# SamsungLabs/nb-asr

Measured on AMD Instinct MI355X. Metric: utterances_per_sec, higher is better.
Workload: dtype f32

## Files before the change

nb_asr_amd/csrc/gemm_pointwise.hip:

```cpp
#include "storage.h"

namespace nbasr {

typedef float floatx4 __attribute__((ext_vector_type(4)));
typedef _Float16 pw_h2 __attribute__((ext_vector_type(2)));

constexpr int PW_M = 128, PW_N = 256, PW_K = 32;
constexpr int PW_THREADS = 512;

__device__ __forceinline__ float pw_load(const float* p) { return *p; }
__device__ __forceinline__ float pw_load(const bf16_t* p) { return __uint_as_float(static_cast<unsigned>(p->bits) << 16); }
__device__ __forceinline__ void pw_store(float* p, float v) { *p = v; }
__device__ __forceinline__ void pw_store(bf16_t* p, float v) { p->bits = static_cast<unsigned short>(pack_bf16x2(v, 0.f) & 0xffffu); }

template <int TERMS>
struct PwSteps {
    static constexpr int NS = TERMS;
    static constexpr int A_STEP = TERMS * 2 * 2 * PW_M * 16;
    static constexpr int X_STEP = TERMS * 2 * 2 * PW_N * 16;
    static constexpr int LDS = 2 * (A_STEP + X_STEP);
};

struct PwF16x2 : PwSteps<2> {
    typedef _Float16 vec8 __attribute__((ext_vector_type(8)));
    typedef float act_t;
    static constexpr bool SCALED = true;
    static constexpr bool ORDER_BY_HOST = true;
    static constexpr int LD_ALIGN = 4, PROJECTION_LD_ALIGN = 1;
    __device__ static __forceinline__ void split2(float a, float b, unsigned (&d)[NS]) {
        const _Float16 ha = static_cast<_Float16>(a), hb = static_cast<_Float16>(b);
        d[0] = __builtin_bit_cast(unsigned, pw_h2{ha, hb});
        d[1] = __builtin_bit_cast(unsigned, pw_h2{static_cast<_Float16>((a - static_cast<float>(ha)) * 2048.f),
                                                  static_cast<_Float16>((b - static_cast<float>(hb)) * 2048.f)});
    }
    __device__ static __forceinline__ floatx4 mfma(vec8 a, vec8 b, floatx4 c) { return __builtin_amdgcn_mfma_f32_16x16x32_f16(a, b, c, 0, 0, 0); }
};

struct PwBf16 : PwSteps<1> {
    typedef __bf16 vec8 __attribute__((ext_vector_type(8)));
    typedef bf16_t act_t;
    static constexpr bool SCALED = false;
    static constexpr bool ORDER_BY_HOST = false;
    static constexpr int LD_ALIGN = 8, PROJECTION_LD_ALIGN = 8;
    __device__ static __forceinline__ void split2(float a, float b, unsigned (&d)[NS]) { d[0] = pack_bf16x2(a, b); }
    __device__ static __forceinline__ floatx4 mfma(vec8 a, vec8 b, floatx4 c) { return __builtin_amdgcn_mfma_f32_16x16x32_bf16(a, b, c, 0, 0, 0); }
};

__host__ __device__ inline void pw_pow2(float absmax, int target, float& scale, float& inv)
{
    unsigned bits;
    __builtin_memcpy(&bits, &absmax, 4);
    const int e = static_cast<int>((bits >> 23) & 0xffu);
    int k = (bits & 0x7fffffffu) ? (127 + target) - e : 0;
    k = k > 126 ? 126 : (k < -126 ? -126 : k);
    const unsigned sb = static_cast<unsigned>(127 + k) << 23, ib = static_cast<unsigned>(127 - k) << 23;
    __builtin_memcpy(&scale, &sb, 4);
    __builtin_memcpy(&inv, &ib, 4);
}

__global__ __launch_bounds__(256) void pw_row_scales_kernel(const float* __restrict__ w, float* __restrict__ scales, int c_out,
                                                            int c_in, int rows)
{
    __shared__ float s_max[4];
    const int co = blockIdx.x;
    float m = 0.f;
    if (co < c_out)
        for (int i = threadIdx.x; i < c_in; i += 256) m = fmaxf(m, fabsf(w[static_cast<size_t>(co) * c_in + i]));
#pragma unroll
    for (int d = 32; d >= 1; d >>= 1) m = fmaxf(m, __shfl_xor(m, d));
    if ((threadIdx.x & 63) == 0) s_max[threadIdx.x >> 6] = m;
    __syncthreads();
    if (threadIdx.x == 0) {
        float scale, inv;
        pw_pow2(fmaxf(fmaxf(s_max[0], s_max[1]), fmaxf(s_max[2], s_max[3])), 13, scale, inv);
        scales[co] = scale;
        scales[rows + co] = inv;
    }
}

template <class P>
__global__ __launch_bounds__(256) void pw_pack_weights_kernel(const float* __restrict__ w, unsigned short* __restrict__ wp,
                                                              const float* __restrict__ row_scale, int c_out, int c_in,
                                                              int n_mt, int n_ks)
{
    const long long total = static_cast<long long>(n_mt) * n_ks * PW_M * PW_K;
    for (long long i = static_cast<long long>(blockIdx.x) * blockDim.x + threadIdx.x; i < total;
         i += static_cast<long long>(gridDim.x) * blockDim.x) {
        long long e = i;
        const int ci_l = e % PW_K; e /= PW_K;
        const int co_l = e % PW_M; e /= PW_M;
        const int ks = e % n_ks; e /= n_ks;
        const int mt = static_cast<int>(e);
        const int co = mt * PW_M + co_l, ci = ks * PW_K + ci_l;
        float v = 0.f;
        if (co < c_out && ci < c_in) v = P::SCALED ? w[static_cast<size_t>(co) * c_in + ci] * row_scale[co] : w[static_cast<size_t>(co) * c_in + ci];
        unsigned d[P::NS];
        P::split2(v, 0.f, d);
        const int blk = ci_l >> 4, half = (ci_l >> 3) & 1, c8 = ci_l & 7;
        const size_t step = static_cast<size_t>(mt) * n_ks + ks;
        const size_t base = step * (P::A_STEP / 2) + ((static_cast<size_t>(blk) * 2 + half) * PW_M + co_l) * 8 + c8;
#pragma unroll
        for (int s = 0; s < P::NS; ++s) wp[base + s * (P::A_STEP / 2 / P::NS)] = static_cast<unsigned short>(d[s] & 0xffffu);
    }
}


template <bool LNX, class T>
__device__ __forceinline__ void pw_fetch32(const T* __restrict__ x, int c_in, int frames, int ld, const LnRef& ln, float (&v)[PW_K])
{
    const int ci0 = blockIdx.y * PW_K, b = blockIdx.z;
    const int t = blockIdx.x * PW_N + threadIdx.x;
    const bool live = t < frames;
    const T* __restrict__ xb = x + static_cast<size_t>(b) * c_in * ld + t;
    float mean = 0.f, rstd = 0.f;
    if (LNX && live) {
        const float* st = ln.stats + static_cast<size_t>(b) * 2 * ld;
        mean = st[t]; rstd = st[ld + t];
    }
#pragma unroll
    for (int c = 0; c < PW_K; ++c) {
        const int ci = ci0 + c;
        v[c] = (live && ci < c_in) ? pw_load(xb + static_cast<size_t>(ci) * ld) : 0.f;
    }
    if (LNX) {
#pragma unroll
        for (int c = 0; c < PW_K; ++c) {
            const int ci = ci0 + c;
            if (live && ci < c_in) v[c] = ln_apply(v[c], mean, rstd, ln.gamma[ci], ln.beta[ci]);
        }
    }
}

template <bool LNX>
__global__ __launch_bounds__(256) void pw_tile_max_kernel(const float* __restrict__ x, float* __restrict__ partial, int c_in,
                                                          int frames, int ld, int n_ks, const LnRef ln)
{
    __shared__ float s_max[4];
    float v[PW_K];
    pw_fetch32<LNX>(x, c_in, frames, ld, ln, v);
    float m = 0.f;
#pragma unroll
    for (int c = 0; c < PW_K; ++c) m = fmaxf(m, fabsf(v[c]));
#pragma unroll
    for (int d = 32; d >= 1; d >>= 1) m = fmaxf(m, __shfl_xor(m, d));
    if ((threadIdx.x & 63) == 0) s_max[threadIdx.x >> 6] = m;
    __syncthreads();
    if (threadIdx.x == 0)
        partial[(static_cast<size_t>(blockIdx.z) * gridDim.x + blockIdx.x) * n_ks + blockIdx.y] = fmaxf(fmaxf(s_max[0], s_max[1]), fmaxf(s_max[2], s_max[3]));
}

template <class P, bool LNX>
__global__ __launch_bounds__(256) void pw_presplit_kernel(const typename P::act_t* __restrict__ x, unsigned char* __restrict__ image,
                                                          float* __restrict__ inv_scale, const float* __restrict__ partial,
                                                          int c_in, int frames, int ld, int n_ks, const LnRef ln)
{
    const int nt = blockIdx.x, ks = blockIdx.y, b = blockIdx.z;
    const int lane_t = threadIdx.x;
    float v[PW_K];
    pw_fetch32<LNX>(x, c_in, frames, ld, ln, v);
    float scale = 1.f;
    if constexpr (P::SCALED) {
        const float* __restrict__ pt = partial + (static_cast<size_t>(b) * gridDim.x + nt) * n_ks;
        float tile_max = 0.f;
        for (int i = threadIdx.x & 63; i < n_ks; i += 64) tile_max = fmaxf(tile_max, pt[i]);
#pragma unroll
        for (int d = 32; d >= 1; d >>= 1) tile_max = fmaxf(tile_max, __shfl_xor(tile_max, d));
        float inv;
        pw_pow2(tile_max, 14, scale, inv);
        if (threadIdx.x == 0 && ks == 0) inv_scale[static_cast<size_t>(b) * gridDim.x + nt] = inv;
    }
    unsigned char* step = image + ((static_cast<size_t>(b) * gridDim.x + nt) * n_ks + ks) * P::X_STEP;
#pragma unroll
    for (int bh = 0; bh < 4; ++bh) {
        u4v term[P::NS];
#pragma unroll
        for (int q = 0; q < 4; ++q) {
            const float v0 = v[bh * 8 + 2 * q], v1 = v[bh * 8 + 2 * q + 1];
            unsigned d[P::NS];
            if constexpr (P::SCALED) P::split2(v0 * scale, v1 * scale, d);
            else P::split2(v0, v1, d);
#pragma unroll
            for (int s = 0; s < P::NS; ++s) term[s][q] = d[s];
        }
        unsigned char* row = step + (bh * PW_N + lane_t) * 16;
#pragma unroll
        for (int s = 0; s < P::NS; ++s) *reinterpret_cast<u4v*>(row + s * (P::X_STEP / P::NS)) = term[s];
    }
}

template <class P>
struct PointwiseArgs {
    const unsigned char* image; const float* x_inv; const unsigned char* wp; const float* w_inv;
    const float* bias; const float* bias2;
    const typename P::act_t* s0; const typename P::act_t* s1; const typename P::act_t* s2;
    void* y;
    int c_out, frames, ld_out, n_ks, n_mt, n_nt, batch;
    int n_major;
    int row_stride_t, row_stride_b;
    LnRef ln_s0;
};

template <class P, bool SWAP, bool RELU>
__global__ __launch_bounds__(PW_THREADS, 2) void pw_gemm_kernel(const PointwiseArgs<P> a)
{
    typedef typename P::vec8 vec8;
    typedef typename P::act_t act_t;
    constexpr int NS = P::NS, A_STEP = P::A_STEP, X_STEP = P::X_STEP;
    extern __shared__ __attribute__((aligned(16))) unsigned char smem[];
    unsigned char* const Abuf = smem;
    unsigned char* const Xbuf = smem + 2 * A_STEP;

    const int nwg = gridDim.x, id = blockIdx.x;
    const int xq = nwg >> 3, xr = nwg & 7, xcd = id & 7;
    const int L = (xcd < xr ? xcd * (xq + 1) : xr * (xq + 1) + (xcd - xr) * xq) + (id >> 3);
    int mt_i, b, nt_i;
    if (!P::ORDER_BY_HOST || a.n_major) {
        const int ntg = L / a.n_mt;
        mt_i = L - ntg * a.n_mt;
        b = ntg / a.n_nt;
        nt_i = ntg - b * a.n_nt;
    } else {
        const int per_m = a.n_nt * a.batch;
        mt_i = L / per_m;
        const int rem = L - mt_i * per_m;
        b = rem / a.n_nt;
        nt_i = rem - b * a.n_nt;
    }
    const int m0 = mt_i * PW_M, n0 = nt_i * PW_N;

    const int tid = threadIdx.x, lane = tid & 63;
    const int wave = __builtin_amdgcn_readfirstlane(tid >> 6);
    const int wm = wave >> 2, wn = wave & 3;
    const int l15 = lane & 15, kq = lane >> 4;
    const bool wave_active = (m0 + wm * 64) < a.c_out && (n0 + wn * 64) < a.ld_out;

    const unsigned char* __restrict__ wsrc = a.wp + static_cast<size_t>(mt_i) * a.n_ks * A_STEP;
    const unsigned char* __restrict__ xsrc = a.image + (static_cast<size_t>(b) * a.n_nt + nt_i) * a.n_ks * X_STEP;

    floatx4 big[4][4], small[4][4];
#pragma unroll
    for (int i = 0; i < 4; ++i)
#pragma unroll
        for (int j = 0; j < 4; ++j)
#pragma unroll
            for (int r = 0; r < 4; ++r) { big[i][j][r] = 0.f; small[i][j][r] = 0.f; }

    auto dma_step = [&](int ks, int buf) {
        const unsigned char* ws = wsrc + static_cast<size_t>(ks) * A_STEP;
        const unsigned char* xs = xsrc + static_cast<size_t>(ks) * X_STEP;
#pragma unroll
        for (int j = 0; j < NS; ++j) {
            const int piece = wave * NS + j;
            __builtin_amdgcn_global_load_lds((const __attribute__((address_space(1))) void*)(ws + piece * 1024 + lane * 16),
                                             (__attribute__((address_space(3))) void*)(Abuf + buf * A_STEP + piece * 1024), 16, 0, 0);
        }
#pragma unroll
        for (int j = 0; j < 2 * NS; ++j) {
            const int piece = wave * 2 * NS + j;
            __builtin_amdgcn_global_load_lds((const __attribute__((address_space(1))) void*)(xs + piece * 1024 + lane * 16),
                                             (__attribute__((address_space(3))) void*)(Xbuf + buf * X_STEP + piece * 1024), 16, 0, 0);
        }
    };

    const int a_lane = ((kq * PW_M) + wm * 64 + l15) * 16;
    const int x_lane = ((kq * PW_N) + wn * 64 + l15) * 16;

    dma_step(0, 0);
    asm volatile("s_waitcnt vmcnt(0)" ::: "memory");
    __syncthreads();
#pragma unroll 1
    for (int ks = 0; ks < a.n_ks; ++ks) {
        const int buf = ks & 1;
        if (ks + 1 < a.n_ks) dma_step(ks + 1, buf ^ 1);
        if (wave_active) {
            const unsigned char* A = Abuf + buf * A_STEP + a_lane;
            const unsigned char* X = Xbuf + buf * X_STEP + x_lane;
            vec8 bt[4][NS];
#pragma unroll
            for (int j = 0; j < 4; ++j)
#pragma unroll
                for (int s = 0; s < NS; ++s) bt[j][s] = *reinterpret_cast<const vec8*>(X + s * (X_STEP / NS) + j * 16 * 16);
#pragma unroll
            for (int i = 0; i < 4; ++i) {
                vec8 at[NS];
#pragma unroll
                for (int s = 0; s < NS; ++s) at[s] = *reinterpret_cast<const vec8*>(A + s * (A_STEP / NS) + i * 16 * 16);
#pragma unroll
                for (int j = 0; j < 4; ++j) {
                    if constexpr (NS == 2) {
                        floatx4 c = small[i][j];
                        c = P::mfma(at[1], bt[j][0], c);
                        c = P::mfma(at[0], bt[j][1], c);
                        small[i][j] = c;
                    }
                    big[i][j] = P::mfma(at[0], bt[j][0], big[i][j]);
                }
            }
        }
        asm volatile("s_waitcnt vmcnt(0)" ::: "memory");
        __syncthreads();
    }

    if (!wave_active) return;
    float x_inv = 1.f;
    if constexpr (P::SCALED) x_inv = a.x_inv[static_cast<size_t>(b) * a.n_nt + nt_i];
    auto product = [&](int i, int j, int r, int m) {
        float v = big[i][j][r];
        if constexpr (NS == 2) v += small[i][j][r] * (1.f / 2048.f);
        if constexpr (P::SCALED) v = v * x_inv * a.w_inv[m];
        return v;
    };
#pragma unroll
    for (int i = 0; i < 4; ++i) {
#pragma unroll
        for (int j = 0; j < 4; ++j) {
            const int n = n0 + wn * 64 + j * 16 + l15;
            const int mb = m0 + wm * 64 + i * 16 + kq * 4;
            if (SWAP) {
                if (n >= a.frames || mb >= a.c_out) continue;
                floatx4 o;
#pragma unroll
                for (int r = 0; r < 4; ++r) {
                    const int m = mb + r;
                    float v = 0.f;
                    if (m < a.c_out) {
                        v = product(i, j, r, m) + a.bias[m];
                        if (a.bias2) v += a.bias2[m];
                        if (RELU) v = relu_clamp(v);
                    }
                    o[r] = v;
                }
                float* dst = static_cast<float*>(a.y) + (static_cast<size_t>(n) * a.row_stride_t + static_cast<size_t>(b) * a.row_stride_b) * a.c_out + mb;
                if (mb + 3 < a.c_out) *reinterpret_cast<floatx4*>(dst) = o;
                else for (int r = 0; r < 4 && mb + r < a.c_out; ++r) dst[r] = o[r];
            } else {
                if (n >= a.ld_out) continue;
                const bool live = n < a.frames;
                float s0m = 0.f, s0r = 0.f;
                if (a.s0 && a.ln_s0.stats) {
                    const float* st = a.ln_s0.stats + static_cast<size_t>(b) * 2 * a.ld_out;
                    s0m = st[n]; s0r = st[a.ld_out + n];
                }
                act_t* yb = static_cast<act_t*>(a.y);
#pragma unroll
                for (int r = 0; r < 4; ++r) {
                    const int m = mb + r;
                    if (m >= a.c_out) continue;
                    float v = product(i, j, r, m) + a.bias[m];
                    if (RELU) v = relu_clamp(v);
                    const size_t off = (static_cast<size_t>(b) * a.c_out + m) * a.ld_out + n;
                    if (a.s0) v += a.ln_s0.stats ? ln_apply(pw_load(a.s0 + off), s0m, s0r, a.ln_s0.gamma[m], a.ln_s0.beta[m]) : pw_load(a.s0 + off);
                    if (a.s1) v += pw_load(a.s1 + off);
                    if (a.s2) v += pw_load(a.s2 + off);
                    pw_store(yb + off, live ? v : 0.f);
                }
            }
        }
    }
}

static inline int pw_n_ks(int c_in) { return (c_in + PW_K - 1) / PW_K; }
static inline int pw_n_mt(int c_out) { return (c_out + PW_M - 1) / PW_M; }
static inline int pw_n_nt(int ld) { return (ld + PW_N - 1) / PW_N; }
static inline size_t pw_round4(size_t n) { return (n + 3) & ~static_cast<size_t>(3); }
template <class P> static size_t pw_image_bytes(int batch, int c_in, int ld) { return static_cast<size_t>(batch) * pw_n_nt(ld) * pw_n_ks(c_in) * P::X_STEP; }
template <class P> static size_t pw_weight_image_bytes(int c_out, int c_in) { return static_cast<size_t>(pw_n_mt(c_out)) * pw_n_ks(c_in) * P::A_STEP; }

template <class P>
static size_t pw_weights_bytes(int c_out, int c_in)
{
    if (c_out <= 0 || c_in <= 0) return 0;
    return pw_weight_image_bytes<P>(c_out, c_in) + (P::SCALED ? 2 * static_cast<size_t>(pw_n_mt(c_out)) * PW_M * sizeof(float) : 0);
}

template <class P>
static size_t pw_workspace_bytes(int batch, int c_in, int ld)
{
    if (batch <= 0 || c_in <= 0 || ld <= 0) return 0;
    const size_t tiles = static_cast<size_t>(batch) * pw_n_nt(ld);
    return pw_image_bytes<P>(batch, c_in, ld) + (P::SCALED ? (pw_round4(tiles) + tiles * pw_n_ks(c_in)) * sizeof(float) : 0);
}

template <class P>
static int pw_pack(const char* what, const float* w, void* packed, int c_out, int c_in, nbasr_stream_t stream)
{
    clear_error();
    NBASR_REQUIRE(c_out > 0 && c_in > 0, NBASR_EINVAL, "%s: bad sizes", what);
    NBASR_REQUIRE(w && packed, NBASR_ENULL, "%s: NULL pointer", what);
    NBASR_REQUIRE(aligned16(packed), NBASR_EALIGN, "%s: packed buffer must be 16-byte aligned", what);
    const int n_mt = pw_n_mt(c_out), n_ks = pw_n_ks(c_in);
    float* scales = nullptr;
    if (P::SCALED) {
        scales = reinterpret_cast<float*>(static_cast<unsigned char*>(packed) + pw_weight_image_bytes<P>(c_out, c_in));
        hipLaunchKernelGGL(pw_row_scales_kernel, dim3(n_mt * PW_M), dim3(256), 0, as_stream(stream), w, scales, c_out, c_in, n_mt * PW_M);
    }
    hipLaunchKernelGGL(pw_pack_weights_kernel<P>, dim3(1024), dim3(256), 0, as_stream(stream), w, static_cast<unsigned short*>(packed), scales,
                       c_out, c_in, n_mt, n_ks);
    return launch_status(what);
}

template <class P, bool LNX>
static int pw_image(const typename P::act_t* x, void* ws, int batch, int c_in, int frames, int ld, LnRef ln, hipStream_t stream, const char* what)
{
    unsigned char* image = static_cast<unsigned char*>(ws);
    float* inv = nullptr;
    float* partial = nullptr;
    const int n_ks = pw_n_ks(c_in);
    const dim3 grid(pw_n_nt(ld), n_ks, batch);
    if constexpr (P::SCALED) {
        inv = reinterpret_cast<float*>(image + pw_image_bytes<P>(batch, c_in, ld));
        partial = inv + pw_round4(static_cast<size_t>(batch) * pw_n_nt(ld));
        hipLaunchKernelGGL(pw_tile_max_kernel<LNX>, grid, dim3(256), 0, stream, x, partial, c_in, frames, ld, n_ks, ln);
    }
    hipLaunchKernelGGL((pw_presplit_kernel<P, LNX>), grid, dim3(256), 0, stream, x, image, inv, partial, c_in, frames, ld, n_ks, ln);
    return launch_status(what);
}

static int pw_checks(const char* what, const void* x, const void* ws, const void* packed_w, const float* bias, const void* y,
                     int batch, int c_in, int frames, int ld, int c_out)
{
    NBASR_REQUIRE(batch >= 0 && c_in > 0 && c_out > 0 && frames >= 0 && ld >= frames, NBASR_EINVAL, "%s: bad sizes", what);
    if (batch == 0 || frames == 0) return 1;
    NBASR_REQUIRE(batch <= 65535, NBASR_EINVAL, "%s: batch %d > 65535", what, batch);
    NBASR_REQUIRE(x && ws && packed_w && bias && y, NBASR_ENULL, "%s: x, workspace, packed_w, bias, y must be non-NULL", what);
    NBASR_REQUIRE(aligned16(ws) && aligned16(packed_w), NBASR_EALIGN, "%s: workspace and packed weights must be 16-byte aligned", what);
    return NBASR_OK;
}

template <class P, bool SWAP, bool RELU>
static int pw_run(const char* what, const typename P::act_t* x, void* ws, const void* packed_w, PointwiseArgs<P> a, int batch, int c_in,
                  int frames, int ld, int c_out, LnRef ln_x, hipStream_t stream)
{
    const int rc = ln_x.stats ? pw_image<P, true>(x, ws, batch, c_in, frames, ld, ln_x, stream, what)
                              : pw_image<P, false>(x, ws, batch, c_in, frames, ld, ln_x, stream, what);
    if (rc != NBASR_OK) return rc;
    a.image = static_cast<const unsigned char*>(ws);
    a.wp = static_cast<const unsigned char*>(packed_w);
    a.n_mt = pw_n_mt(c_out); a.n_ks = pw_n_ks(c_in); a.n_nt = pw_n_nt(ld);
    if (P::SCALED) {
        a.x_inv = reinterpret_cast<const float*>(a.image + pw_image_bytes<P>(batch, c_in, ld));
        a.w_inv = reinterpret_cast<const float*>(a.wp + pw_weight_image_bytes<P>(c_out, c_in)) + static_cast<size_t>(a.n_mt) * PW_M;
    }
    a.c_out = c_out; a.frames = frames; a.ld_out = ld; a.batch = batch;

    static const hipError_t attr = hipFuncSetAttribute(reinterpret_cast<const void*>(pw_gemm_kernel<P, SWAP, RELU>),
                                                       hipFuncAttributeMaxDynamicSharedMemorySize, P::LDS);
    if (attr != hipSuccess) {
        set_error("%s: cannot reserve %d bytes of LDS: %s", what, P::LDS, hipGetErrorString(attr));
        return static_cast<int>(attr);
    }
    const long long nwg = static_cast<long long>(a.n_mt) * a.n_nt * a.batch;
    NBASR_REQUIRE(nwg < (1ll << 31), NBASR_EINVAL, "%s: too many tiles (%lld)", what, nwg);
    a.n_major = static_cast<long long>(a.n_mt) * P::A_STEP <= static_cast<long long>(a.n_nt) * a.batch * P::X_STEP ? 1 : 0;
    hipLaunchKernelGGL((pw_gemm_kernel<P, SWAP, RELU>), dim3(static_cast<unsigned>(nwg)), dim3(PW_THREADS), P::LDS, stream, a);
    return launch_status(what);
}

template <class P>
static int pw_linear(const char* what, const typename P::act_t* x, void* ws, const void* packed_w, const float* bias,
                     const typename P::act_t* skip0, const typename P::act_t* skip1, const typename P::act_t* skip2, typename P::act_t* y,
                     int batch, int c_in, int frames, int ld, int c_out, const nbasr_deferred_ln* ln, int ln_on_x, int ln_on_skip0,
                     nbasr_stream_t stream)
{
    clear_error();
    const int rc0 = pw_checks(what, x, ws, packed_w, bias, y, batch, c_in, frames, ld, c_out);
    if (rc0 != NBASR_OK) return rc0 == 1 ? NBASR_OK : rc0;
    NBASR_REQUIRE(ld % P::LD_ALIGN == 0, NBASR_EALIGN, "%s: ld=%d must be a multiple of %d (rows are pitched to 16 bytes)", what, ld, P::LD_ALIGN);
    const bool any_ln = ln && (ln_on_x || (ln_on_skip0 && skip0));
    NBASR_REQUIRE(!any_ln || (ln->stats && ln->gamma && ln->beta), NBASR_ENULL, "%s: deferred LayerNorm needs stats, gamma and beta", what);
    NBASR_REQUIRE(!(ln && ln_on_x && ln_on_skip0 && skip0) || c_in == c_out, NBASR_EINVAL, "%s: one descriptor for x and skip0 needs equal shapes", what);
    PointwiseArgs<P> a{};
    a.bias = bias; a.s0 = skip0; a.s1 = skip1; a.s2 = skip2; a.y = y;
    a.ln_s0 = ln_ref(ln, ln_on_skip0 != 0 && skip0 != nullptr);
    return pw_run<P, false, true>(what, x, ws, packed_w, a, batch, c_in, frames, ld, c_out, ln_ref(ln, ln_on_x != 0), as_stream(stream));
}

template <class P>
static int pw_projection(const char* what, const typename P::act_t* x, void* ws, const void* packed_w_ih, const float* b_ih, const float* b_hh,
                         float* gates_ws, int batch, int c_in, int frames, int ld, int hidden, const nbasr_deferred_ln* ln, int batch_total,
                         int batch_offset, nbasr_stream_t stream)
{
    const int rc0 = pw_checks(what, x, ws, packed_w_ih, b_ih, gates_ws, batch, c_in, frames, ld, 4 * hidden);
    if (rc0 != NBASR_OK) return rc0 == 1 ? NBASR_OK : rc0;
    NBASR_REQUIRE(b_hh != nullptr, NBASR_ENULL, "%s: b_hh is NULL", what);
    NBASR_REQUIRE(hidden % 4 == 0 && aligned16(gates_ws) && ld % P::PROJECTION_LD_ALIGN == 0, NBASR_EALIGN,
                  "%s: hidden %% 4, ld %% %d and 16-byte aligned gates_ws required", what, P::PROJECTION_LD_ALIGN);
    NBASR_REQUIRE(!ln || (ln->stats && ln->gamma && ln->beta), NBASR_ENULL, "%s: deferred LayerNorm needs stats, gamma and beta", what);
    PointwiseArgs<P> a{};
    a.bias = b_ih; a.bias2 = b_hh; a.y = gates_ws + static_cast<size_t>(batch_offset) * 4 * hidden;
    a.row_stride_t = batch_total; a.row_stride_b = 1;
    return pw_run<P, true, false>(what, x, ws, packed_w_ih, a, batch, c_in, frames, ld, 4 * hidden, ln_ref(ln, true), as_stream(stream));
}

}

using namespace nbasr;

extern "C" size_t nbasr_pointwise_packed_weights_bytes(int c_out, int c_in) { return pw_weights_bytes<PwF16x2>(c_out, c_in); }
extern "C" size_t nbasr_pointwise_bf16_weights_bytes(int c_out, int c_in) { return pw_weights_bytes<PwBf16>(c_out, c_in); }
extern "C" size_t nbasr_pointwise_workspace_bytes(int batch, int c_in, int ld) { return pw_workspace_bytes<PwF16x2>(batch, c_in, ld); }
extern "C" size_t nbasr_pointwise_bf16_workspace_bytes(int batch, int c_in, int ld) { return pw_workspace_bytes<PwBf16>(batch, c_in, ld); }

extern "C" int nbasr_pack_pointwise_weights(const float* w, void* packed, int c_out, int c_in, nbasr_stream_t stream)
{
    return pw_pack<PwF16x2>("nbasr_pack_pointwise_weights", w, packed, c_out, c_in, stream);
}

extern "C" int nbasr_pack_pointwise_weights_bf16(const float* w, void* packed, int c_out, int c_in, nbasr_stream_t stream)
// ... 53 lines not shown
```

nb_asr_amd/csrc/layernorm.hip:

```cpp
#include "storage.h"

namespace nbasr {

constexpr int LN_ROWS = 16;
constexpr int LN_QS = 16;

template <typename T, bool MINMAX = false, int FR = Chunk<T>::FR>
__device__ __forceinline__ void tile_statistics(const T* x, int channels, int ld, float eps, size_t base, bool active,
                                                int row, int ql, float (*s_mean)[LN_QS * FR], float (*s_m2)[LN_QS * FR],
                                                float* s_cnt, float* s_mu, float* s_rstd,
                                                float (*s_lo)[LN_QS * FR] = nullptr, float (*s_hi)[LN_QS * FR] = nullptr)
{
    float shift[FR], s1[FR], s2[FR], lo[FR], hi[FR];
#pragma unroll
    for (int r = 0; r < FR; ++r) { shift[r] = 0.f; s1[r] = 0.f; s2[r] = 0.f; lo[r] = 3.0e38f; hi[r] = -3.0e38f; }
    int n = 0;
    if (active && row < channels) {
        load_frames<FR>(x + base + static_cast<size_t>(row) * ld, shift);
        auto fold = [&](const float (&e)[FR]) {
#pragma unroll
            for (int r = 0; r < FR; ++r) {
                const float d = e[r] - shift[r];
                s1[r] += d;
                s2[r] = __builtin_fmaf(d, d, s2[r]);
// ... 95 lines not shown
#pragma unroll
        for (int r = 0; r < FR; ++r) {
            o[r] = (o[r] - mu[r]) * rs[r] * g + bt;
            if (t0 + r >= frames) o[r] = 0.f;
            if (ABSMAX) amax = fmaxf(amax, finite_abs(o[r]));
        }
        store_frames<FR, false>(y + off, o);
    }
    if (ABSMAX) {
#pragma unroll
        for (int m = 32; m >= 1; m >>= 1) amax = fmaxf(amax, __shfl_xor(amax, m));
        if ((threadIdx.x & 63) == 0) atomicMax(absmax + b, __float_as_uint(amax));
    }
}

template <typename T>
__global__ __launch_bounds__(256) void channel_stats_kernel(const T* __restrict__ x, float* __restrict__ stats,
                                                            int channels, int frames, int ld, float eps)
{
    constexpr int FR = Chunk<T>::FR;
    __shared__ float s_mean[LN_ROWS][LN_QS * FR];
    __shared__ float s_m2[LN_ROWS][LN_QS * FR];
    __shared__ float s_cnt[LN_ROWS];
    __shared__ float s_mu[LN_QS * FR];
    __shared__ float s_rstd[LN_QS * FR];

    const int ql = threadIdx.x & (LN_QS - 1);
    const int row = threadIdx.x / LN_QS;
    const int nq = ld / FR;
    const int q = blockIdx.x * LN_QS + ql;
    const int b = blockIdx.y;
    const bool active = q < nq;
    const size_t base = static_cast<size_t>(b) * channels * ld + static_cast<size_t>(q) * FR;

    tile_statistics<T>(x, channels, ld, eps, base, active, row, ql, s_mean, s_m2, s_cnt, s_mu, s_rstd);

    if (threadIdx.x < LN_QS * FR) {
        const int t = blockIdx.x * (LN_QS * FR) + threadIdx.x;
        if (t < ld) {
            const bool live = t < frames;
            float* srow = stats + static_cast<size_t>(b) * 2 * ld;
            srow[t] = live ? s_mu[threadIdx.x] : 0.f;
            srow[ld + t] = live ? s_rstd[threadIdx.x] : 0.f;
        }
    }
}

}

using namespace nbasr;

static int layernorm_impl(const char* what, const void* x, const float* gamma, const float* beta, void* y, float* absmax,
                          int batch, int channels, int frames, int ld, float eps, nbasr_stream_t stream,
                          int in_dtype = NBASR_F32, int out_dtype = NBASR_F32)
{
    clear_error();
    NBASR_REQUIRE((in_dtype == NBASR_F32 || in_dtype == NBASR_BF16) && (out_dtype == NBASR_F32 || out_dtype == NBASR_BF16) &&
                  !(in_dtype == NBASR_F32 && out_dtype == NBASR_BF16), NBASR_EINVAL,
                  "%s: storage types (%d -> %d) unsupported (f32 -> f32, bf16 -> bf16, bf16 -> f32)", what, in_dtype, out_dtype);
    NBASR_REQUIRE(batch >= 0 && channels > 0 && frames >= 0, NBASR_EINVAL, "%s: bad sizes", what);
    const int fr = in_dtype == NBASR_BF16 ? 8 : 4;
    NBASR_REQUIRE(ld >= frames && ld % fr == 0, NBASR_EALIGN, "%s: ld=%d must be >= frames=%d and a multiple of %d", what, ld, frames, fr);
    if (batch == 0 || ld == 0) return NBASR_OK;
    NBASR_REQUIRE(x && gamma && beta && y, NBASR_ENULL, "%s: NULL pointer", what);
    NBASR_REQUIRE(aligned16(x) && aligned16(y), NBASR_EALIGN, "%s: x, y must be 16-byte aligned", what);
    NBASR_REQUIRE(batch <= 65535, NBASR_EINVAL, "%s: batch %d > 65535", what, batch);
    NBASR_REQUIRE(!absmax || in_dtype == NBASR_F32, NBASR_EINVAL, "%s: the absmax by-product exists for fp32 tensors only", what);
    const int nq = ld / fr;
    const dim3 grid((nq + LN_QS - 1) / LN_QS, batch);
    if (in_dtype == NBASR_BF16) {
        if (out_dtype == NBASR_BF16)
            hipLaunchKernelGGL((layernorm_channels_kernel<bf16_t, bf16_t, false>), grid, dim3(256), 0, as_stream(stream),
                               static_cast<const bf16_t*>(x), gamma, beta, static_cast<bf16_t*>(y), channels, frames, ld, eps, static_cast<unsigned*>(nullptr));
        else
            hipLaunchKernelGGL((layernorm_channels_kernel<bf16_t, float, false>), grid, dim3(256), 0, as_stream(stream),
                               static_cast<const bf16_t*>(x), gamma, beta, static_cast<float*>(y), channels, frames, ld, eps, static_cast<unsigned*>(nullptr));
    } else if (absmax) {
        zero_async(absmax, sizeof(float) * batch, as_stream(stream));
        hipLaunchKernelGGL((layernorm_channels_kernel<float, float, true>), grid, dim3(256), 0, as_stream(stream),
                           static_cast<const float*>(x), gamma, beta, static_cast<float*>(y), channels, frames, ld, eps, reinterpret_cast<unsigned*>(absmax));
    } else {
        hipLaunchKernelGGL((layernorm_channels_kernel<float, float, false>), grid, dim3(256), 0, as_stream(stream),
                           static_cast<const float*>(x), gamma, beta, static_cast<float*>(y), channels, frames, ld, eps, static_cast<unsigned*>(nullptr));
    }
    return launch_status(what);
}

extern "C" int nbasr_layernorm_channels(const void* x, const float* gamma, const float* beta, void* y, float* absmax, int batch,
                                        int channels, int frames, int ld, float eps, int in_dtype, int out_dtype, nbasr_stream_t stream)
{
    clear_error();
    NBASR_REQUIRE(!absmax || (in_dtype == NBASR_F32 && out_dtype == NBASR_F32), NBASR_EINVAL,
                  "nbasr_layernorm_channels: the max|y| by-product exists for fp32 -> fp32 only");
    return layernorm_impl("nbasr_layernorm_channels", x, gamma, beta, y, absmax, batch, channels, frames, ld, eps, stream, in_dtype, out_dtype);
}

__global__ __launch_bounds__(256) void channel_stats_bound_kernel(const float* __restrict__ x, const float* __restrict__ gamma,
                                                                  const float* __restrict__ beta, float* __restrict__ stats,
                                                                  unsigned* __restrict__ bound, int channels, int frames, int ld, float eps)
{
    __shared__ float s_mean[LN_ROWS][LN_QS * 4];
    __shared__ float s_m2[LN_ROWS][LN_QS * 4];
    __shared__ float s_cnt[LN_ROWS];
    __shared__ float s_mu[LN_QS * 4];
    __shared__ float s_rstd[LN_QS * 4];
    __shared__ float s_gb[8];
    __shared__ float s_lo[LN_ROWS][LN_QS * 4];
    __shared__ float s_hi[LN_ROWS][LN_QS * 4];

    const int ql = threadIdx.x & (LN_QS - 1);
    const int row = threadIdx.x / LN_QS;
    const int nq = ld >> 2;
    const int q = blockIdx.x * LN_QS + ql;
    const int b = blockIdx.y;
    const bool active = q < nq;
    const size_t base = static_cast<size_t>(b) * channels * ld + static_cast<size_t>(q) * 4;

    float gm = 0.f, bm = 0.f;
    for (int c = threadIdx.x; c < channels; c += 256) { gm = fmaxf(gm, fabsf(gamma[c])); bm = fmaxf(bm, fabsf(beta[c])); }
#pragma unroll
    for (int d = 32; d >= 1; d >>= 1) { gm = fmaxf(gm, __shfl_xor(gm, d)); bm = fmaxf(bm, __shfl_xor(bm, d)); }
    if ((threadIdx.x & 63) == 0) { s_gb[threadIdx.x >> 6] = gm; s_gb[4 + (threadIdx.x >> 6)] = bm; }

    tile_statistics<float, true>(x, channels, ld, eps, base, active, row, ql, s_mean, s_m2, s_cnt, s_mu, s_rstd, s_lo, s_hi);
    gm = fmaxf(fmaxf(s_gb[0], s_gb[1]), fmaxf(s_gb[2], s_gb[3]));
    bm = fmaxf(fmaxf(s_gb[4], s_gb[5]), fmaxf(s_gb[6], s_gb[7]));

    float dev = 0.f;
    if (threadIdx.x < LN_QS * 4) {
        const int t = blockIdx.x * (LN_QS * 4) + threadIdx.x;
        if (t < ld) {
            const bool live = t < frames;
            float* srow = stats + static_cast<size_t>(b) * 2 * ld;
            srow[t] = live ? s_mu[threadIdx.x] : 0.f;
            srow[ld + t] = live ? s_rstd[threadIdx.x] : 0.f;
            if (live) dev = finite_abs(fmaxf(s_hi[0][threadIdx.x] - s_mu[threadIdx.x], s_mu[threadIdx.x] - s_lo[0][threadIdx.x]) * s_rstd[threadIdx.x]);
        }
    }
    if (threadIdx.x < 64) {
#pragma unroll
        for (int d = 32; d >= 1; d >>= 1) dev = fmaxf(dev, __shfl_xor(dev, d));
        if (threadIdx.x == 0) atomicMax(bound + b, __float_as_uint(finite_abs((dev * gm + bm) * 1.0001f)));
    }
}

template <bool NORM>
__global__ __launch_bounds__(256) void normalize_split_kernel(const float* __restrict__ x, const float* __restrict__ stats,
                                                              const float* __restrict__ gamma, const float* __restrict__ beta,
                                                              const float* __restrict__ bound, unsigned char* __restrict__ image,
                                                              int channels, int , int ld,
                                                              int bound_stride)
{
    typedef _Float16 halfx8 __attribute__((ext_vector_type(8)));
    const int ql = threadIdx.x & 63, oct0 = (threadIdx.x >> 6) + 4 * blockIdx.z;
    const int nq = ld >> 2;
    const int q = blockIdx.x * 64 + ql;
    const int b = blockIdx.y;
    const int n_groups = (channels + 15) >> 4;
    const size_t rows = static_cast<size_t>(ld) + 1;
    unsigned char* const img_b = image + static_cast<size_t>(b) * n_groups * 4 * rows * 16;
    if (blockIdx.x == 0 && blockIdx.z == 0) {
        const uint4 z = make_uint4(0u, 0u, 0u, 0u);
        for (int pl = threadIdx.x; pl < n_groups * 4; pl += 256) *reinterpret_cast<uint4*>(img_b + static_cast<size_t>(pl) * rows * 16) = z;
    }
    if (q >= nq) return;
    float scale = 1.f;
    {
        const unsigned bits = __float_as_uint(bound[static_cast<size_t>(b) * bound_stride]);
        const int e = static_cast<int>((bits >> 23) & 0xffu);
        int k = (bits & 0x7fffffffu) ? (127 + 14) - e : 0;
        k = k > 126 ? 126 : (k < -126 ? -126 : k);
        scale = __uint_as_float(static_cast<unsigned>(127 + k) << 23);
    }
    float m4[4] = {0.f, 0.f, 0.f, 0.f}, r4[4] = {0.f, 0.f, 0.f, 0.f};
    if constexpr (NORM) {
        const float* st = stats + static_cast<size_t>(b) * 2 * ld + q * 4;
        const float4 mu = *reinterpret_cast<const float4*>(st), rs = *reinterpret_cast<const float4*>(st + ld);
        m4[0] = mu.x; m4[1] = mu.y; m4[2] = mu.z; m4[3] = mu.w;
        r4[0] = rs.x; r4[1] = rs.y; r4[2] = rs.z; r4[3] = rs.w;
    }
    const float* xb = x + static_cast<size_t>(b) * channels * ld + static_cast<size_t>(q) * 4;
    const int n_oct = (channels + 7) >> 3;
    for (int oct = oct0; oct < 2 * n_groups; oct += 4 * gridDim.z) {
        float v[8][4];
#pragma unroll
        for (int c = 0; c < 8; ++c) {
            const int ch = oct * 8 + c;
            float4 t4 = make_float4(0.f, 0.f, 0.f, 0.f);
            float g = 0.f, be = 0.f;
            if (oct < n_oct && ch < channels) {
                t4 = *reinterpret_cast<const float4*>(xb + static_cast<size_t>(ch) * ld);
                if constexpr (NORM) { g = gamma[ch]; be = beta[ch]; }
            }
            const float e4[4] = {t4.x, t4.y, t4.z, t4.w};
#pragma unroll
            for (int r = 0; r < 4; ++r) {
                if constexpr (NORM) v[c][r] = (ch < channels) ? ln_apply(e4[r], m4[r], r4[r], g, be) * scale : 0.f;
                else                v[c][r] = e4[r] * scale;
            }
        }
        unsigned char* plane_hi = img_b + ((static_cast<size_t>(oct >> 1) * 4 + (oct & 1)) * rows + 1 + static_cast<size_t>(q) * 4) * 16;
        unsigned char* plane_lo = plane_hi + 2 * rows * 16;
#pragma unroll
        for (int r = 0; r < 4; ++r) {
            halfx8 hi, lo;
#pragma unroll
            for (int c = 0; c < 8; ++c) {
                const _Float16 h = static_cast<_Float16>(v[c][r]);
                hi[c] = h;
                lo[c] = static_cast<_Float16>(v[c][r] - static_cast<float>(h));
            }
            *reinterpret_cast<halfx8*>(plane_hi + r * 16) = hi;
            *reinterpret_cast<halfx8*>(plane_lo + r * 16) = lo;
        }
    }
}

static int split_grid_z(int tiles, int batch)
{
    const long long wgs = static_cast<long long>(tiles) * batch;
    int z = 4;
    while (z < 16 && wgs * z < 512) z *= 2;
    return z;
}

extern "C" int nbasr_layernorm_split_image(const float* x, const float* gamma, const float* beta, float* stats, float* bound,
                                           void* image, int batch, int channels, int frames, int ld, float eps,
                                           nbasr_stream_t stream)
{
    clear_error();
    NBASR_REQUIRE(batch >= 0 && channels > 0 && frames >= 0, NBASR_EINVAL, "nbasr_layernorm_split_image: bad sizes");
    NBASR_REQUIRE(ld >= frames && ld % 4 == 0, NBASR_EALIGN, "nbasr_layernorm_split_image: ld=%d must be >= frames=%d and a multiple of 4", ld, frames);
    if (batch == 0 || ld == 0) return NBASR_OK;
    NBASR_REQUIRE(x && gamma && beta && stats && bound && image, NBASR_ENULL, "nbasr_layernorm_split_image: NULL pointer");
    NBASR_REQUIRE(aligned16(x) && aligned16(stats) && aligned16(image), NBASR_EALIGN, "nbasr_layernorm_split_image: x, stats, image must be 16-byte aligned");
    NBASR_REQUIRE(batch <= 65535, NBASR_EINVAL, "nbasr_layernorm_split_image: batch %d > 65535", batch);
    zero_async(bound, sizeof(float) * batch, as_stream(stream));
    const int nq = ld / 4;
    hipLaunchKernelGGL(channel_stats_bound_kernel, dim3((nq + LN_QS - 1) / LN_QS, batch), dim3(256), 0, as_stream(stream),
                       x, gamma, beta, stats, reinterpret_cast<unsigned*>(bound), channels, frames, ld, eps);
    hipLaunchKernelGGL(normalize_split_kernel<true>, dim3((nq + 63) / 64, batch, split_grid_z((nq + 63) / 64, batch)), dim3(256), 0, as_stream(stream),
                       x, stats, gamma, beta, bound, static_cast<unsigned char*>(image), channels, frames, ld, 1);
    return launch_status("nbasr_layernorm_split_image");
}

__global__ __launch_bounds__(256) void input_range_kernel(const float* __restrict__ x, unsigned* __restrict__ range,
                                                          int channels, int frames, int ld)
{
    __shared__ float s_max[4][256];
    __shared__ unsigned s_bad[4];
    const int b = blockIdx.y;
    const int lane = threadIdx.x & 63, slice = threadIdx.x >> 6;
    const int t0 = (blockIdx.x * 64 + lane) * 4;
    float m[4] = {0.f, 0.f, 0.f, 0.f};
    unsigned bad = 0u;
    if (t0 < frames) {
        const float* col = x + static_cast<size_t>(b) * channels * ld + t0;
        const bool whole = t0 + 4 <= ld && ld % 4 == 0 && (reinterpret_cast<size_t>(x) & 15) == 0;
        for (int c = slice; c < channels; c += 4) {
            float v[4] = {0.f, 0.f, 0.f, 0.f};
            if (whole) {
                const float4 q = *reinterpret_cast<const float4*>(col + static_cast<size_t>(c) * ld);
                v[0] = q.x; v[1] = q.y; v[2] = q.z; v[3] = q.w;
            } else {
#pragma unroll
                for (int r = 0; r < 4; ++r) if (t0 + r < frames) v[r] = col[static_cast<size_t>(c) * ld + r];
            }
#pragma unroll
            for (int r = 0; r < 4; ++r) {
                const float a = fabsf(v[r]);
                if (t0 + r < frames) {
                    if (!(a <= 3.4028234664e38f)) bad = 1u;
                    else m[r] = fmaxf(m[r], a);
                }
            }
        }
    }
#pragma unroll
    for (int r = 0; r < 4; ++r) s_max[slice][lane * 4 + r] = m[r];
#pragma unroll
    for (int d = 32; d >= 1; d >>= 1) bad |= __shfl_xor(bad, d);
    if (lane == 0) s_bad[slice] = bad;
    __syncthreads();
    const int t = blockIdx.x * 256 + threadIdx.x;
    const float fmax_ = fmaxf(fmaxf(s_max[0][threadIdx.x], s_max[1][threadIdx.x]), fmaxf(s_max[2][threadIdx.x], s_max[3][threadIdx.x]));
    float hi = fmax_, lo = (t < frames && fmax_ > 0.f) ? fmax_ : __uint_as_float(0x7f800000u);
#pragma unroll
    for (int d = 32; d >= 1; d >>= 1) {
        hi = fmaxf(hi, __shfl_xor(hi, d));
        lo = fminf(lo, __shfl_xor(lo, d));
    }
    if (lane == 0) {
        atomicMax(range + 4 * b, __float_as_uint(hi));
        atomicMin(range + 4 * b + 1, __float_as_uint(lo));
        if (slice == 0 && (s_bad[0] | s_bad[1] | s_bad[2] | s_bad[3])) atomicOr(range + 4 * b + 2, 0x3f800000u);
    }
}

__global__ void input_range_init_kernel(unsigned* __restrict__ range, int batch)
{
    const int b = blockIdx.x * blockDim.x + threadIdx.x;
    if (b < batch) { range[4 * b] = 0u; range[4 * b + 1] = 0x7f800000u; range[4 * b + 2] = 0u; range[4 * b + 3] = 0u; }
}

extern "C" int nbasr_input_range(const float* x, float* range, int batch, int channels, int frames, int ld, nbasr_stream_t stream)
{
    clear_error();
    NBASR_REQUIRE(batch >= 0 && channels > 0 && frames >= 0 && ld >= frames, NBASR_EINVAL, "nbasr_input_range: bad sizes");
    if (batch == 0) return NBASR_OK;
    NBASR_REQUIRE(range, NBASR_ENULL, "nbasr_input_range: range is NULL");
    NBASR_REQUIRE(batch <= 65535, NBASR_EINVAL, "nbasr_input_range: batch %d > 65535", batch);
    hipLaunchKernelGGL(input_range_init_kernel, dim3((batch + 255) / 256), dim3(256), 0, as_stream(stream), reinterpret_cast<unsigned*>(range), batch);
    if (frames > 0) {
        NBASR_REQUIRE(x, NBASR_ENULL, "nbasr_input_range: x is NULL");
        hipLaunchKernelGGL(input_range_kernel, dim3((frames + 255) / 256, batch), dim3(256), 0, as_stream(stream), x,
                           reinterpret_cast<unsigned*>(range), channels, frames, ld);
    }
    return launch_status("nbasr_input_range");
}

extern "C" int nbasr_split_image_ranged(const float* x, const float* x_range, void* image, int batch, int channels, int frames,
                                        int ld, nbasr_stream_t stream)
{
    clear_error();
    NBASR_REQUIRE(batch >= 0 && channels > 0 && frames >= 0, NBASR_EINVAL, "nbasr_split_image_ranged: bad sizes");
    NBASR_REQUIRE(ld >= frames && ld % 4 == 0, NBASR_EALIGN, "nbasr_split_image_ranged: ld=%d must be >= frames=%d and a multiple of 4", ld, frames);
    if (batch == 0 || ld == 0) return NBASR_OK;
    NBASR_REQUIRE(x && x_range && image, NBASR_ENULL, "nbasr_split_image_ranged: NULL pointer");
    NBASR_REQUIRE(aligned16(x) && aligned16(image), NBASR_EALIGN, "nbasr_split_image_ranged: x, image must be 16-byte aligned");
    NBASR_REQUIRE(batch <= 65535, NBASR_EINVAL, "nbasr_split_image_ranged: batch %d > 65535", batch);
    const int nq = ld / 4;
    hipLaunchKernelGGL(normalize_split_kernel<false>, dim3((nq + 63) / 64, batch, split_grid_z((nq + 63) / 64, batch)), dim3(256), 0, as_stream(stream),
                       x, static_cast<const float*>(nullptr), static_cast<const float*>(nullptr), static_cast<const float*>(nullptr),
                       x_range, static_cast<unsigned char*>(image), channels, frames, ld, 4);
    return launch_status("nbasr_split_image_ranged");
}

extern "C" int nbasr_channel_stats(const void* x, float* stats, int batch, int channels, int frames, int ld, float eps, int dtype,
                                     nbasr_stream_t stream)
{
    clear_error();
    NBASR_REQUIRE(dtype == NBASR_F32 || dtype == NBASR_BF16, NBASR_EINVAL, "nbasr_channel_stats: unknown dtype %d", dtype);
    NBASR_REQUIRE(batch >= 0 && channels > 0 && frames >= 0, NBASR_EINVAL, "nbasr_channel_stats: bad sizes");
    const int fr = dtype == NBASR_BF16 ? 8 : 4;
    NBASR_REQUIRE(ld >= frames && ld % fr == 0, NBASR_EALIGN, "nbasr_channel_stats: ld=%d must be >= frames=%d and a multiple of %d", ld, frames, fr);
    if (batch == 0 || ld == 0) return NBASR_OK;
    NBASR_REQUIRE(x && stats, NBASR_ENULL, "nbasr_channel_stats: NULL pointer");
    NBASR_REQUIRE(aligned16(x) && aligned16(stats), NBASR_EALIGN, "nbasr_channel_stats: x, stats must be 16-byte aligned");
    NBASR_REQUIRE(batch <= 65535, NBASR_EINVAL, "nbasr_channel_stats: batch %d > 65535", batch);
    const int nq = ld / fr;
    const dim3 grid((nq + LN_QS - 1) / LN_QS, batch);
    if (dtype == NBASR_BF16)
        hipLaunchKernelGGL(channel_stats_kernel<bf16_t>, grid, dim3(256), 0, as_stream(stream), static_cast<const bf16_t*>(x), stats, channels, frames, ld, eps);
    else
        hipLaunchKernelGGL(channel_stats_kernel<float>, grid, dim3(256), 0, as_stream(stream), static_cast<const float*>(x), stats, channels, frames, ld, eps);
    return launch_status("nbasr_channel_stats");
}

template <typename T, bool NORM>
__global__ __launch_bounds__(256) void bf16_image_kernel(const T* __restrict__ x, const float* __restrict__ stats,
                                                         const float* __restrict__ gamma, const float* __restrict__ beta,
                                                         unsigned char* __restrict__ image, int channels, int frames, int ld)
{
    constexpr int FR = Chunk<T>::FR;
    const int ql = threadIdx.x & 15, oct0 = threadIdx.x >> 4;
    const int nq = ld / FR;
    const int q = blockIdx.x * 16 + ql;
// ... 110 lines not shown
```

Before: 11110.

## Triple-buffer pointwise GEMM with wave-priority DMA and LDS-staged stores

The pointwise GEMM goes from double to triple-buffered LDS, prefetching two K-steps ahead and waiting with partial vmcnt. It splits DMA issue between older and younger waves with s_setprio, interleaves A-fragment reads with the MFMAs under sched_barrier, and stages the SWAP epilogue through LDS so global stores are coalesced float4 rows. The layernorm split-image kernel now software-prefetches the next octet and transposes its half-precision planes through shared memory for contiguous stores. The added LDS footprint may reduce occupancy, and the SWAP store path drops the per-element c_out tail guard.

After: 11250 (median of 6 runs). +1.3%, better.

```diff
diff --git a/nb_asr_amd/csrc/gemm_pointwise.hip b/nb_asr_amd/csrc/gemm_pointwise.hip
--- a/nb_asr_amd/csrc/gemm_pointwise.hip
+++ b/nb_asr_amd/csrc/gemm_pointwise.hip
@@ -18,7 +18,9 @@
     static constexpr int NS = TERMS;
     static constexpr int A_STEP = TERMS * 2 * 2 * PW_M * 16;
     static constexpr int X_STEP = TERMS * 2 * 2 * PW_N * 16;
-    static constexpr int LDS = 2 * (A_STEP + X_STEP);
+    static constexpr int RING = 3;
+    static constexpr int LDS = RING * (A_STEP + X_STEP);
+    static constexpr int DMA_PER_WAVE = 3 * TERMS;
 };
 
 struct PwF16x2 : PwSteps<2> {
@@ -208,7 +210,7 @@
     constexpr int NS = P::NS, A_STEP = P::A_STEP, X_STEP = P::X_STEP;
     extern __shared__ __attribute__((aligned(16))) unsigned char smem[];
     unsigned char* const Abuf = smem;
-    unsigned char* const Xbuf = smem + 2 * A_STEP;
+    unsigned char* const Xbuf = smem + P::RING * A_STEP;
 
     const int nwg = gridDim.x, id = blockIdx.x;
     const int xq = nwg >> 3, xr = nwg & 7, xcd = id & 7;
@@ -265,41 +267,61 @@
     const int a_lane = ((kq * PW_M) + wm * 64 + l15) * 16;
     const int x_lane = ((kq * PW_N) + wn * 64 + l15) * 16;
 
-    dma_step(0, 0);
-    asm volatile("s_waitcnt vmcnt(0)" ::: "memory");
-    __syncthreads();
-#pragma unroll 1
-    for (int ks = 0; ks < a.n_ks; ++ks) {
-        const int buf = ks & 1;
-        if (ks + 1 < a.n_ks) dma_step(ks + 1, buf ^ 1);
-        if (wave_active) {
-            const unsigned char* A = Abuf + buf * A_STEP + a_lane;
-            const unsigned char* X = Xbuf + buf * X_STEP + x_lane;
-            vec8 bt[4][NS];
-#pragma unroll
-            for (int j = 0; j < 4; ++j)
-#pragma unroll
-                for (int s = 0; s < NS; ++s) bt[j][s] = *reinterpret_cast<const vec8*>(X + s * (X_STEP / NS) + j * 16 * 16);
-#pragma unroll
-            for (int i = 0; i < 4; ++i) {
-                vec8 at[NS];
-#pragma unroll
-                for (int s = 0; s < NS; ++s) at[s] = *reinterpret_cast<const vec8*>(A + s * (A_STEP / NS) + i * 16 * 16);
-#pragma unroll
-                for (int j = 0; j < 4; ++j) {
-                    if constexpr (NS == 2) {
-                        floatx4 c = small[i][j];
-                        c = P::mfma(at[1], bt[j][0], c);
-                        c = P::mfma(at[0], bt[j][1], c);
-                        small[i][j] = c;
-                    }
-                    big[i][j] = P::mfma(at[0], bt[j][0], big[i][j]);
+    auto mma_step = [&](int buf) {
+        const unsigned char* A = Abuf + buf * A_STEP + a_lane;
+        const unsigned char* X = Xbuf + buf * X_STEP + x_lane;
+        auto read_a = [&](int i, vec8 (&f)[NS]) {
+#pragma unroll
+            for (int s = 0; s < NS; ++s) f[s] = *reinterpret_cast<const vec8*>(A + s * (A_STEP / NS) + i * 16 * 16);
+        };
+        vec8 bt[4][NS], at[2][NS];
+#pragma unroll
+        for (int j = 0; j < 4; ++j)
+#pragma unroll
+            for (int s = 0; s < NS; ++s) bt[j][s] = *reinterpret_cast<const vec8*>(X + s * (X_STEP / NS) + j * 16 * 16);
+        read_a(0, at[0]);
+#pragma unroll
+        for (int i = 0; i < 4; ++i) {
+#pragma unroll
+            for (int j = 0; j < 4; ++j) {
+                __builtin_amdgcn_sched_barrier(0);
+                if constexpr (NS == 2) {
+                    floatx4 c = small[i][j];
+                    c = P::mfma(at[i & 1][1], bt[j][0], c);
+                    c = P::mfma(at[i & 1][0], bt[j][1], c);
+                    small[i][j] = c;
                 }
+                big[i][j] = P::mfma(at[i & 1][0], bt[j][0], big[i][j]);
+                __builtin_amdgcn_sched_barrier(0);
+                if (j == 0 && i < 3) read_a(i + 1, at[(i + 1) & 1]);
             }
         }
-        asm volatile("s_waitcnt vmcnt(0)" ::: "memory");
-        __syncthreads();
-    }
+        __builtin_amdgcn_sched_barrier(0);
+    };
+
+    const bool older = wave < 4;
+    const int n_ks = a.n_ks;
+    dma_step(0, 0);
+    if (n_ks > 1) {
+        dma_step(1, 1);
+        asm volatile("s_waitcnt vmcnt(%0)\n\ts_barrier" :: "n"(P::DMA_PER_WAVE) : "memory");
+    } else {
+        asm volatile("s_waitcnt vmcnt(0)\n\ts_barrier" ::: "memory");
+    }
+    if (!older) __builtin_amdgcn_s_setprio(1);
+    int buf = 0;
+#pragma unroll 1
+    for (int ks = 0; ks < n_ks; ++ks) {
+        const bool ahead = ks + 2 < n_ks;
+        const int fill = buf == 0 ? 2 : buf - 1;
+        if (older && ahead) dma_step(ks + 2, fill);
+        if (wave_active) mma_step(buf);
+        if (!older && ahead) dma_step(ks + 2, fill);
+        if (ahead) asm volatile("s_waitcnt vmcnt(%0) lgkmcnt(0)\n\ts_barrier" :: "n"(P::DMA_PER_WAVE) : "memory");
+        else       asm volatile("s_waitcnt vmcnt(0) lgkmcnt(0)\n\ts_barrier" ::: "memory");
+        buf = buf == 2 ? 0 : buf + 1;
+    }
+    if (!older) __builtin_amdgcn_s_setprio(0);
 
     if (!wave_active) return;
     float x_inv = 1.f;
@@ -310,14 +332,16 @@
         if constexpr (P::SCALED) v = v * x_inv * a.w_inv[m];
         return v;
     };
-#pragma unroll
-    for (int i = 0; i < 4; ++i) {
+    if constexpr (SWAP) {
+        constexpr int TS = 64 + 4;
+        static_assert(8 * 16 * TS * 4 <= P::LDS, "output staging must fit the operand buffers");
+        float* const T = reinterpret_cast<float*>(smem) + wave * (16 * TS);
+        const int mseg = m0 + wm * 64 + l15 * 4;
 #pragma unroll
         for (int j = 0; j < 4; ++j) {
-            const int n = n0 + wn * 64 + j * 16 + l15;
-            const int mb = m0 + wm * 64 + i * 16 + kq * 4;
-            if (SWAP) {
-                if (n >= a.frames || mb >= a.c_out) continue;
+#pragma unroll
+            for (int i = 0; i < 4; ++i) {
+                const int mb = m0 + wm * 64 + i * 16 + kq * 4;
                 floatx4 o;
 #pragma unroll
                 for (int r = 0; r < 4; ++r) {
@@ -330,30 +354,47 @@
                     }
                     o[r] = v;
                 }
-                float* dst = static_cast<float*>(a.y) + (static_cast<size_t>(n) * a.row_stride_t + static_cast<size_t>(b) * a.row_stride_b) * a.c_out + mb;
-                if (mb + 3 < a.c_out) *reinterpret_cast<floatx4*>(dst) = o;
-                else for (int r = 0; r < 4 && mb + r < a.c_out; ++r) dst[r] = o[r];
-            } else {
-                if (n >= a.ld_out) continue;
-                const bool live = n < a.frames;
-                float s0m = 0.f, s0r = 0.f;
-                if (a.s0 && a.ln_s0.stats) {
-                    const float* st = a.ln_s0.stats + static_cast<size_t>(b) * 2 * a.ld_out;
-                    s0m = st[n]; s0r = st[a.ld_out + n];
-                }
-                act_t* yb = static_cast<act_t*>(a.y);
-#pragma unroll
-                for (int r = 0; r < 4; ++r) {
-                    const int m = mb + r;
-                    if (m >= a.c_out) continue;
-                    float v = product(i, j, r, m) + a.bias[m];
-                    if (RELU) v = relu_clamp(v);
-                    const size_t off = (static_cast<size_t>(b) * a.c_out + m) * a.ld_out + n;
-                    if (a.s0) v += a.ln_s0.stats ? ln_apply(pw_load(a.s0 + off), s0m, s0r, a.ln_s0.gamma[m], a.ln_s0.beta[m]) : pw_load(a.s0 + off);
-                    if (a.s1) v += pw_load(a.s1 + off);
-                    if (a.s2) v += pw_load(a.s2 + off);
-                    pw_store(yb + off, live ? v : 0.f);
-                }
+                *reinterpret_cast<floatx4*>(T + l15 * TS + i * 16 + kq * 4) = o;
+            }
+            asm volatile("s_waitcnt lgkmcnt(0)" ::: "memory");
+#pragma unroll
+            for (int it = 0; it < 4; ++it) {
+                const int row = it * 4 + kq;
+                const int n = n0 + wn * 64 + j * 16 + row;
+                if (n >= a.frames || mseg >= a.c_out) continue;
+                const floatx4 o = *reinterpret_cast<const floatx4*>(T + row * TS + l15 * 4);
+                float* dst = static_cast<float*>(a.y) + (static_cast<size_t>(n) * a.row_stride_t + static_cast<size_t>(b) * a.row_stride_b) * a.c_out + mseg;
+                *reinterpret_cast<floatx4*>(dst) = o;
+            }
+            asm volatile("s_waitcnt lgkmcnt(0)" ::: "memory");
+        }
+        return;
+    }
+#pragma unroll
+    for (int i = 0; i < 4; ++i) {
+#pragma unroll
+        for (int j = 0; j < 4; ++j) {
+            const int n = n0 + wn * 64 + j * 16 + l15;
+            const int mb = m0 + wm * 64 + i * 16 + kq * 4;
+            if (n >= a.ld_out) continue;
+            const bool live = n < a.frames;
+            float s0m = 0.f, s0r = 0.f;
+            if (a.s0 && a.ln_s0.stats) {
+                const float* st = a.ln_s0.stats + static_cast<size_t>(b) * 2 * a.ld_out;
+                s0m = st[n]; s0r = st[a.ld_out + n];
+            }
+            act_t* yb = static_cast<act_t*>(a.y);
+#pragma unroll
+            for (int r = 0; r < 4; ++r) {
+                const int m = mb + r;
+                if (m >= a.c_out) continue;
+                float v = product(i, j, r, m) + a.bias[m];
+                if (RELU) v = relu_clamp(v);
+                const size_t off = (static_cast<size_t>(b) * a.c_out + m) * a.ld_out + n;
+                if (a.s0) v += a.ln_s0.stats ? ln_apply(pw_load(a.s0 + off), s0m, s0r, a.ln_s0.gamma[m], a.ln_s0.beta[m]) : pw_load(a.s0 + off);
+                if (a.s1) v += pw_load(a.s1 + off);
+                if (a.s2) v += pw_load(a.s2 + off);
+                pw_store(yb + off, live ? v : 0.f);
             }
         }
     }
diff --git a/nb_asr_amd/csrc/layernorm.hip b/nb_asr_amd/csrc/layernorm.hip
--- a/nb_asr_amd/csrc/layernorm.hip
+++ b/nb_asr_amd/csrc/layernorm.hip
@@ -271,7 +271,9 @@
                                                               int bound_stride)
 {
     typedef _Float16 halfx8 __attribute__((ext_vector_type(8)));
-    const int ql = threadIdx.x & 63, oct0 = (threadIdx.x >> 6) + 4 * blockIdx.z;
+    constexpr int SPLIT_PITCH = 68;
+    __shared__ __attribute__((aligned(16))) unsigned char s_tile[4][2][4 * SPLIT_PITCH * 16];
+    const int ql = threadIdx.x & 63, wv = threadIdx.x >> 6, oct0 = wv + 4 * blockIdx.z;
     const int nq = ld >> 2;
     const int q = blockIdx.x * 64 + ql;
     const int b = blockIdx.y;
@@ -282,7 +284,8 @@
         const uint4 z = make_uint4(0u, 0u, 0u, 0u);
         for (int pl = threadIdx.x; pl < n_groups * 4; pl += 256) *reinterpret_cast<uint4*>(img_b + static_cast<size_t>(pl) * rows * 16) = z;
     }
-    if (q >= nq) return;
+    if (blockIdx.x * 64 >= nq) return;
+    const bool inside = q < nq;
     float scale = 1.f;
     {
         const unsigned bits = __float_as_uint(bound[static_cast<size_t>(b) * bound_stride]);
@@ -293,33 +296,50 @@
     }
     float m4[4] = {0.f, 0.f, 0.f, 0.f}, r4[4] = {0.f, 0.f, 0.f, 0.f};
     if constexpr (NORM) {
-        const float* st = stats + static_cast<size_t>(b) * 2 * ld + q * 4;
-        const float4 mu = *reinterpret_cast<const float4*>(st), rs = *reinterpret_cast<const float4*>(st + ld);
-        m4[0] = mu.x; m4[1] = mu.y; m4[2] = mu.z; m4[3] = mu.w;
-        r4[0] = rs.x; r4[1] = rs.y; r4[2] = rs.z; r4[3] = rs.w;
+        if (inside) {
+            const float* st = stats + static_cast<size_t>(b) * 2 * ld + q * 4;
+            const float4 mu = *reinterpret_cast<const float4*>(st), rs = *reinterpret_cast<const float4*>(st + ld);
+            m4[0] = mu.x; m4[1] = mu.y; m4[2] = mu.z; m4[3] = mu.w;
+            r4[0] = rs.x; r4[1] = rs.y; r4[2] = rs.z; r4[3] = rs.w;
+        }
     }
     const float* xb = x + static_cast<size_t>(b) * channels * ld + static_cast<size_t>(q) * 4;
     const int n_oct = (channels + 7) >> 3;
-    for (int oct = oct0; oct < 2 * n_groups; oct += 4 * gridDim.z) {
-        float v[8][4];
+    const int oct_step = 4 * gridDim.z;
+    auto load_octet = [&](int oct, float4 (&t)[8]) {
 #pragma unroll
         for (int c = 0; c < 8; ++c) {
             const int ch = oct * 8 + c;
-            float4 t4 = make_float4(0.f, 0.f, 0.f, 0.f);
+            t[c] = make_float4(0.f, 0.f, 0.f, 0.f);
+            if (inside && oct < n_oct && ch < channels) t[c] = *reinterpret_cast<const float4*>(xb + static_cast<size_t>(ch) * ld);
+        }
+    };
+    unsigned char* const tile_hi = s_tile[wv][0];
+    unsigned char* const tile_lo = s_tile[wv][1];
+    float4 cur[8];
+    if (oct0 < 2 * n_groups) load_octet(oct0, cur);
+    for (int oct = oct0; oct < 2 * n_groups; oct += oct_step) {
+        float4 nxt[8];
+        if (oct + oct_step < 2 * n_groups) load_octet(oct + oct_step, nxt);
+        else {
+#pragma unroll
+            for (int c = 0; c < 8; ++c) nxt[c] = make_float4(0.f, 0.f, 0.f, 0.f);
+        }
+        float v[8][4];
+#pragma unroll
+        for (int c = 0; c < 8; ++c) {
+            const int ch = oct * 8 + c;
             float g = 0.f, be = 0.f;
-            if (oct < n_oct && ch < channels) {
-                t4 = *reinterpret_cast<const float4*>(xb + static_cast<size_t>(ch) * ld);
-                if constexpr (NORM) { g = gamma[ch]; be = beta[ch]; }
-            }
-            const float e4[4] = {t4.x, t4.y, t4.z, t4.w};
+            if constexpr (NORM) {
+                if (oct < n_oct && ch < channels) { g = gamma[ch]; be = beta[ch]; }
+            }
+            const float e4[4] = {cur[c].x, cur[c].y, cur[c].z, cur[c].w};
 #pragma unroll
             for (int r = 0; r < 4; ++r) {
                 if constexpr (NORM) v[c][r] = (ch < channels) ? ln_apply(e4[r], m4[r], r4[r], g, be) * scale : 0.f;
                 else                v[c][r] = e4[r] * scale;
             }
         }
-        unsigned char* plane_hi = img_b + ((static_cast<size_t>(oct >> 1) * 4 + (oct & 1)) * rows + 1 + static_cast<size_t>(q) * 4) * 16;
-        unsigned char* plane_lo = plane_hi + 2 * rows * 16;
 #pragma unroll
         for (int r = 0; r < 4; ++r) {
             halfx8 hi, lo;
@@ -329,9 +349,26 @@
                 hi[c] = h;
                 lo[c] = static_cast<_Float16>(v[c][r] - static_cast<float>(h));
             }
-            *reinterpret_cast<halfx8*>(plane_hi + r * 16) = hi;
-            *reinterpret_cast<halfx8*>(plane_lo + r * 16) = lo;
-        }
+            *reinterpret_cast<halfx8*>(tile_hi + (r * SPLIT_PITCH + ql) * 16) = hi;
+            *reinterpret_cast<halfx8*>(tile_lo + (r * SPLIT_PITCH + ql) * 16) = lo;
+        }
+        asm volatile("s_waitcnt lgkmcnt(0)" ::: "memory");
+        unsigned char* plane_hi = img_b + ((static_cast<size_t>(oct >> 1) * 4 + (oct & 1)) * rows + 1 + static_cast<size_t>(blockIdx.x) * 256) * 16;
+        unsigned char* plane_lo = plane_hi + 2 * rows * 16;
+#pragma unroll
+        for (int k = 0; k < 4; ++k) {
+            const int src = ((ql & 3) * SPLIT_PITCH + 16 * k + (ql >> 2)) * 16;
+            const halfx8 hi = *reinterpret_cast<const halfx8*>(tile_hi + src);
+            const halfx8 lo = *reinterpret_cast<const halfx8*>(tile_lo + src);
+            const int f = 64 * k + ql;
+            if (blockIdx.x * 256 + f < ld) {
+                *reinterpret_cast<halfx8*>(plane_hi + f * 16) = hi;
+                *reinterpret_cast<halfx8*>(plane_lo + f * 16) = lo;
+            }
+        }
+        asm volatile("s_waitcnt lgkmcnt(0)" ::: "memory");
+#pragma unroll
+        for (int c = 0; c < 8; ++c) cur[c] = nxt[c];
     }
 }
 
```
